# wgurecky/CORRLA_RS

Hardware: AMD Instinct MI355X
Metric: RSVD GFLOP/s on 16k x 16k f32 rank-128 (higher is better)
Workload: dtype f32

## Files before the change

### corrla_rs_amd/csrc/gemm_plan.hpp

```cpp
#pragma once
#include <algorithm>
#include <cstddef>
#include <cstdint>

#include "core_svd_plan.hpp"

namespace corrla {

constexpr int kMaxColTiles = 9;

struct ColBlocking {
  int tiles, nblk, nt;
  int64_t cols_alloc;
};
inline ColBlocking col_blocking(int64_t cols) {
  ColBlocking b;
  b.tiles = (int)std::max<int64_t>(1, (cols + 15) / 16);
  b.nblk = (b.tiles + kMaxColTiles - 1) / kMaxColTiles;
  b.nt = (b.tiles + b.nblk - 1) / b.nblk;
  b.cols_alloc = (int64_t)b.nblk * b.nt * 16;
  return b;
}

namespace k {

constexpr int kRowBytes = 256;
constexpr int kLoaders = 4;
CORRLA_HD constexpr int gemm_vec(int esz) { return 16 / esz; }
CORRLA_HD constexpr int gemm_kt(int esz) { return kRowBytes / esz; }
CORRLA_HD constexpr int outer_tile(int mw) { return 64 * mw; }
CORRLA_HD constexpr int big_tile_bytes(int mw) { return 64 * 256 * mw; }
CORRLA_HD constexpr int stage_bytes(int mw, int nt) { return big_tile_bytes(mw) + nt * 16 * kRowBytes; }
CORRLA_HD constexpr int gemm_stages(int mw, int nt) { return 3 * stage_bytes(mw, nt) <= 160 * 1024 ? 3 : 2; }
CORRLA_HD constexpr int gemm_lds_bytes(int mw, int nt) { return gemm_stages(mw, nt) * stage_bytes(mw, nt); }

template <class T>
CORRLA_HD constexpr int gram_rows() { return 512 / (int)sizeof(T); }
CORRLA_HD constexpr int gram_tile_bytes(int nct) { return 16 * nct * 512; }
CORRLA_HD constexpr int gram_stages(int nct) {
  const int s = (160 * 1024 - 4096) / gram_tile_bytes(nct);
  return s > 4 ? 4 : s;
}
CORRLA_HD constexpr int gram_lds_bytes(int nct, int esz) {
  const int ring = gram_stages(nct) * gram_tile_bytes(nct);
  const int red = 3 * (nct * (nct + 1) / 2) * 256 * esz;
  return ring > red ? ring : red;
}

constexpr int kMxWaves = 8;
constexpr int kMxLoaders = 4;
constexpr int kMxRowTiles = 2;
constexpr int kMxOuter = kMxWaves * kMxRowTiles * 16;
constexpr int kMxKT = 32;
constexpr int kMxBigBytes = kMxOuter * kMxKT * 4;
CORRLA_HD constexpr int mx_plane_bytes(int nt) { return nt * 16 * kMxKT * 2; }
constexpr int kMxASlots = 3, kMxBSlots = 2;
CORRLA_HD constexpr int mx_bslot_bytes(int nt, int np) { return np * mx_plane_bytes(nt); }
CORRLA_HD constexpr int mx_lds_bytes(int nt, int np) { return kMxASlots * kMxBigBytes + kMxBSlots * mx_bslot_bytes(nt, np) + 1024; }

}

struct GemmKnobs {
  int split_nn = 0, split_tn = 0;
  int mw = 0;
  int xcd_remap = 1;
  int64_t tall_min_rows = 65536;
  int persist_max_tiles = 16;
  int f64_waves = 8;
  double mixed_min_work = 16777216.0;
  bool even_blocks = false;
  bool no_gram_alias = false;
  bool no_rotate = false;
  int mixed_split = 0;
};

struct GemmOperand {
  int64_t rows = 0, cols = 0, ld = 0, cols_readable = 0, cols_alloc = 0;
  bool external = false, aligned = true;
};
struct GemmShape {
  bool tn = false;
  int esz = 4;
  GemmOperand r, x, out;
  bool same = false;
  int np = 0;
  int num_cus = 256;
};

enum class GemmFamily { general, gram_alias, tall_apply, tall_gram, bf16_split };
enum class SlabReduce { none, plain, deep };

struct SlabReducePlan {
  SlabReduce kind = SlabReduce::none;
  unsigned grid[2] = {0, 0};
  int slabs = 0;
  int64_t rows = 0, cols = 0;
};

struct GemmLaunch {
  unsigned grid[3] = {1, 1, 1};
  int nt = 0;
  int64_t col_base = 0;
  int xcd_remap = 0;
  int lds = 0;
};

struct GemmPlan {
  const char* error = nullptr;
  GemmFamily family = GemmFamily::general;
  int mw = 1, nw = 4, np = 0;
  int block = 256;
  int nlaunch = 0;
  GemmLaunch launch[2];
  int tiles_total = 0, nsplit = 1, tiles_per_split = 0, outer_blocks = 0, rotate = 0, vec_store = 0;
  int64_t out_cols = 0;
  int64_t slab_stride = 0;
  size_t slab_bytes = 0;
  SlabReducePlan reduce;
  int64_t rows_per_group = 0, groups = 0;
  int64_t plane_stride = 0, plane_cols = 0;
  size_t plane_bytes = 0;
  unsigned split_grid = 0;
};

inline bool gemm_mixed_domain(const GemmShape& s, const GemmKnobs& kn) {
  const int64_t outer_n = s.tn ? s.r.cols : s.r.rows, red_n = s.tn ? s.r.rows : s.r.cols;
  if (s.esz != 4 || s.x.external || col_blocking(s.x.cols).nblk != 1) return false;
  if (!s.r.aligned || (s.r.ld % 4) || (s.r.cols_readable % 4) || !s.x.aligned || (s.x.ld % 64)) return false;
  if (s.x.ld < (red_n + k::kMxKT - 1) / k::kMxKT * k::kMxKT || s.out.ld < outer_n || s.out.rows != outer_n) return false;
  if (s.same) return false;
  return outer_n >= 1 && red_n >= 1 && (double)outer_n * (double)red_n >= kn.mixed_min_work;
}

namespace gemm_plan_detail {

inline bool grid_fits(unsigned y, unsigned z) { return y <= 65535u && z <= 65535u; }
inline bool padding_fits(const GemmShape& s, const ColBlocking& cb) {
  return cb.cols_alloc <= s.x.cols_alloc && (s.out.external ? s.out.cols >= s.x.cols : cb.cols_alloc <= s.out.cols_alloc);
}
inline GemmPlan rejected(GemmPlan p, const char* why) {
  p.error = why;
  return p;
}

inline bool plan_reduce(GemmPlan& p, int64_t outer_n, int64_t cols_alloc) {
  if (p.nsplit <= 1) return true;
  const bool deep = p.nsplit >= 8;
  const unsigned rows_per_wg = deep ? 64 : 256;
  p.reduce = {deep ? SlabReduce::deep : SlabReduce::plain,
// ... 117 lines not shown
      nsplit = (int)((s.num_cus + wgs - 1) / wgs);
      if (wgs * nsplit < 2 * (int64_t)s.num_cus && wgs < s.num_cus / 4) nsplit *= 2;
      nsplit = std::min(nsplit, std::max(1, p.tiles_total / 4));
    }
    nsplit = std::min(std::max(1, std::min(nsplit, p.tiles_total)), 65535);
  }
  const int64_t outer_tiles = (outer_n + 64 * mw - 1) / (64 * mw);
  if (outer_tiles > 0x7fffffff) return rejected(p, "outer dimension too large");

  p.family = alias ? GemmFamily::gram_alias : GemmFamily::general;
  p.mw = mw == 2 ? 2 : 1;
  if (!alias && mw == 2 && s.esz == 8 && kn.f64_waves == 8) {
    p.mw = 1;
    p.nw = 8;
  }
  p.block = 64 * (p.nw + k::kLoaders);
  p.nsplit = nsplit;
  p.tiles_per_split = (p.tiles_total + nsplit - 1) / nsplit;
  p.outer_blocks = (int)outer_tiles;
  p.out_cols = s.out.external ? s.out.cols : (uneven ? (int64_t)cb.tiles * 16 : cb.cols_alloc);
  p.vec_store = ((s.out.ld % 4) == 0 && s.out.aligned) ? 1 : 0;
  p.rotate = (!s.tn && !alias && p.tiles_per_split <= 32 && p.tiles_per_split > 1 && !kn.no_rotate) ? 1 : 0;
  p.slab_stride = s.out.ld * cb.cols_alloc;
  if (nsplit > 1) p.slab_bytes = (size_t)nsplit * (size_t)p.slab_stride * s.esz;

  int64_t gx = outer_tiles;
  if (!alias && p.tiles_per_split <= kn.persist_max_tiles) {
    const int64_t lds_full = (int64_t)k::gemm_lds_bytes(mw, cb.nt);
    const int64_t per_cu = std::max<int64_t>(1, std::min<int64_t>(4, (160 * 1024) / lds_full));
    const int64_t slots = per_cu * s.num_cus / ((int64_t)cb.nblk * nsplit);
    if (slots >= 1 && outer_tiles >= 3 * slots) gx = slots;
  }
  if (!grid_fits((unsigned)cb.nblk, (unsigned)nsplit)) return rejected(p, "problem too large for the launch grid");

  const int gw = p.mw * p.nw / 4;
  p.nlaunch = uneven ? 2 : 1;
  for (int i = 0; i < p.nlaunch; ++i) {
    GemmLaunch& L = p.launch[i];
    L.grid[0] = (unsigned)gx;
    L.grid[1] = (unsigned)(uneven ? (i == 0 ? n_wide : cb.nblk - n_wide) : cb.nblk);
    L.grid[2] = (unsigned)nsplit;
    L.nt = cb.nt - i;
    L.col_base = (int64_t)i * n_wide * cb.nt * 16;
    L.xcd_remap = (s.tn && kn.xcd_remap && L.grid[1] == 1 && gx == outer_tiles && outer_tiles >= 2 && outer_tiles <= 32 &&
                   nsplit >= 8) ? 1 : 0;
    if (alias) {
      L.lds = 3 * k::big_tile_bytes(2);
    } else {
      const int64_t per_wg = (int64_t)std::max(1, p.tiles_per_split) * ((outer_tiles + gx - 1) / gx);
      L.lds = (int)std::min<int64_t>(k::gemm_stages(gw, L.nt), per_wg) * k::stage_bytes(gw, L.nt);
    }
  }
  if (!plan_reduce(p, outer_n, cb.cols_alloc)) p.error = "problem too large for the launch grid";
  return p;
}

}
```

### corrla_rs_amd/csrc/hip_backend.hpp

```cpp
#pragma once
#include <hip/hip_runtime.h>
#include <rccl/rccl.h>

#include <cmath>
#include <cstdio>
#include <cstdlib>
#include <cstring>
#include <limits>
#include <random>
#include <string>
#include <type_traits>
#include <vector>

#include "core_svd_plan.hpp"
#include "driver.hpp"
#include "hip_kernels.hpp"
#include "tsqr_kernels.hpp"
#include "jacobi_mc_kernels.hpp"
#include "ata_kernels.hpp"
#include "tall_kernels.hpp"
#include "mixed_kernels.hpp"
#include "grad_kernels.hpp"
#include "knn2_kernels.hpp"
#include "grad_wide_kernels.hpp"
// ... 29 lines not shown
struct NcclType<double> {
  static constexpr ncclDataType_t v = ncclDouble;
};

class HipDev {
 public:
  int device = 0;
  int num_cus = 256;
  hipStream_t stream = nullptr;
  ncclComm_t comm = nullptr;
  int comm_rank = 0, comm_size = 1;
  int n_collectives = 0;
  double collective_bytes = 0;

  explicit HipDev(int dev_ordinal) : device(dev_ordinal) {
    int count = 0;
    if (hipGetDeviceCount(&count) != hipSuccess || count <= 0)
      throw Error(ST_ENODEV, "no HIP device visible (libcorrla_rsvd has no CPU fallback)");
    if (dev_ordinal < 0 || dev_ordinal >= count) throw Error(ST_EINVAL, "device ordinal out of range");
    CORRLA_HIP(hipSetDevice(device));
    hipDeviceProp_t prop;
    CORRLA_HIP(hipGetDeviceProperties(&prop, device));
    if (std::strncmp(prop.gcnArchName, "gfx950", 6) != 0)
      throw Error(ST_ENODEV, std::string("device is ") + prop.gcnArchName + ", this library is built for gfx950 only");
    num_cus = prop.multiProcessorCount;
    CORRLA_HIP(hipStreamCreateWithFlags(&stream, hipStreamNonBlocking));
    CORRLA_HIP(hipMalloc(&zero_page_, 256));
    CORRLA_HIP(hipHostMalloc(&pinned_, kPinnedBytes, hipHostMallocDefault));
    for (auto& e : events_) CORRLA_HIP(hipEventCreate(&e));
    CORRLA_HIP(hipMemsetAsync(zero_page_, 0, 256, stream));
    set_lds_limits();
    {
      std::random_device rd;
      entropy_ = ((uint64_t)rd() << 32) ^ (uint64_t)rd();
    }
    no_device_chol_ = env_int("CORRLA_HOST_CHOL", 0) != 0;
    jmc_min_l_ = env_int("CORRLA_JMC_MIN_L", 96);
    jmc_max_b_ = std::min(32, std::max(2, env_int("CORRLA_JMC_MAX_B", 24)));
    robust_passes_ = std::max(2, env_int("CORRLA_ROBUST_PASSES", 2));
    robust_qr_ = env_int("CORRLA_DEVICE_ROBUST_QR", 1) != 0;
    gemm_debug_flags_ = env_int("CORRLA_GEMM_DEBUG", 0);
    gemm_knobs_.split_nn = env_int("CORRLA_SPLIT_NN", 0);
    gemm_knobs_.split_tn = env_int("CORRLA_SPLIT_TN", 0);
    gemm_knobs_.mw = env_int("CORRLA_MW", 0);
    gemm_knobs_.xcd_remap = env_int("CORRLA_GEMM_XCD", 1);
    gemm_knobs_.tall_min_rows = env_int("CORRLA_TALL_MIN_ROWS", 65536);
    gemm_knobs_.persist_max_tiles = env_int("CORRLA_GEMM_PERSIST_TILES", 16);
    gemm_knobs_.f64_waves = env_int("CORRLA_F64_WAVES", 8);
    if (const char* e = std::getenv("CORRLA_MIXED_MIN_WORK")) gemm_knobs_.mixed_min_work = std::atof(e);
    gemm_knobs_.even_blocks = env_int("CORRLA_EVEN_BLOCKS", 0) != 0;
    gemm_knobs_.no_gram_alias = env_int("CORRLA_NO_GRAM_ALIAS", 0) != 0;
    gemm_knobs_.no_rotate = env_int("CORRLA_GEMM_NO_ROTATE", 0) != 0;
    gemm_knobs_.mixed_split = env_int("CORRLA_MIXED_SPLIT", 0);
  }
  ~HipDev() {
    (void)hipSetDevice(device);
    if (stream) (void)hipStreamSynchronize(stream);
    if (comm) (void)ncclCommDestroy(comm);
    for (auto& c : chunks_) (void)hipFree(c.p);
    for (auto& c : zchunks_) (void)hipFree(c.p);
    if (zero_page_) (void)hipFree(zero_page_);
    if (pinned_) (void)hipHostFree(pinned_);
    for (auto& e : events_)
      if (e) (void)hipEventDestroy(e);
    for (auto& e : ev_pool_) (void)hipEventDestroy(e);
    if (stream) (void)hipStreamDestroy(stream);
  }
  HipDev(const HipDev&) = delete;
  HipDev& operator=(const HipDev&) = delete;

  int nranks() const { return comm_size; }

  uint64_t fresh_seed(bool rank_invariant) {
    uint64_t z = (rank_invariant ? 0x5eedull : entropy_) + 0x9e3779b97f4a7c15ull * (uint64_t)(++(rank_invariant ? calls_sharded_ : calls_));
    z = (z ^ (z >> 30)) * 0xbf58476d1ce4e5b9ull;
    z = (z ^ (z >> 27)) * 0x94d049bb133111ebull;
    z ^= z >> 31;
    return z ? z : 0x5eedull;
  }

  void comm_init(const void* id128, int rank, int nranks_) {
    CORRLA_HIP(hipSetDevice(device));
    ncclUniqueId id;
    static_assert(sizeof(ncclUniqueId) <= CORRLA_UNIQUE_ID_BYTES, "unique id size");
    std::memcpy(&id, id128, sizeof(id));
    if (comm) {
      (void)ncclCommDestroy(comm);
      comm = nullptr;
    }
    CORRLA_NCCL(ncclCommInitRank(&comm, nranks_, id, rank));
    comm_rank = rank;
    comm_size = nranks_;
  }
  void comm_info(int* rank_out, int* nranks_out) {
    if (!comm) {
      *rank_out = 0;
      *nranks_out = 0;
      return;
    }
    CORRLA_NCCL(ncclCommUserRank(comm, rank_out));
    CORRLA_NCCL(ncclCommCount(comm, nranks_out));
  }

  void begin_call() {
    CORRLA_HIP(hipSetDevice(device));
    events_set_[0] = events_set_[1] = events_set_[2] = false;
    n_collectives = 0;
    collective_bytes = 0;
    marks_.clear();
    ev_used_ = 0;
    phase_mark(nullptr);
    for (auto& c : chunks_) c.used = 0;
    sp_scratch_ = nullptr;
    sp_scratch_bytes_ = 0;
    for (auto& c : zchunks_) {
      c.zeroed = std::min<size_t>(c.used, (size_t)256 << 20);
      c.used = 0;
      if (c.zeroed) CORRLA_HIP(hipMemsetAsync(c.p, 0, c.zeroed, stream));
    }
  }
  void end_call() { sync(); }
  void sync() { CORRLA_HIP(hipStreamSynchronize(stream)); }

  void* alloc_bytes(size_t bytes) {
    bytes = (bytes + 255) / 256 * 256;
    if (bytes == 0) bytes = 256;
    for (auto& c : chunks_)
      if (c.size - c.used >= bytes) {
        void* p = (char*)c.p + c.used;
        c.used += bytes;
        return p;
      }
    Chunk c;
    c.size = std::max<size_t>(bytes, (size_t)64 << 20);
    if (hipMalloc(&c.p, c.size) != hipSuccess) {
      (void)hipGetLastError();
      throw Error(ST_ENOMEM, "device allocation of " + std::to_string(c.size) + " bytes failed");
    }
    c.used = bytes;
    chunks_.push_back(c);
    return c.p;
  }
  void memset_zero(void* p, size_t bytes) { CORRLA_HIP(hipMemsetAsync(p, 0, bytes, stream)); }
  void* alloc_zeroed(size_t bytes) {
    bytes = (bytes + 255) / 256 * 256;
    if (bytes == 0) bytes = 256;
    Chunk* hit = nullptr;
    for (auto& c : zchunks_)
      if (c.size - c.used >= bytes) {
        hit = &c;
        break;
      }
    if (!hit) {
      Chunk c;
      c.size = std::max<size_t>(bytes, (size_t)128 << 20);
      if (hipMalloc(&c.p, c.size) != hipSuccess) {
        (void)hipGetLastError();
        throw Error(ST_ENOMEM, "device allocation of " + std::to_string(c.size) + " bytes failed");
      }
      zchunks_.push_back(c);
      hit = &zchunks_.back();
    }
    char* p = (char*)hit->p + hit->used;
    const size_t end = hit->used + bytes;
    if (end > hit->zeroed) {
      const size_t from = std::max(hit->used, hit->zeroed);
      CORRLA_HIP(hipMemsetAsync((char*)hit->p + from, 0, end - from, stream));
    }
    hit->used = end;
    return p;
  }

  template <class T>
  Skinny<T> alloc_skinny(int64_t rows, int64_t cols) {
    Skinny<T> s;
    s.rows = rows;
    s.cols = cols;
    s.ld = round_up(std::max<int64_t>(rows, 1), kLdPad);
    s.cols_alloc = col_blocking(cols).cols_alloc;
    const size_t bytes = (size_t)s.ld * (size_t)s.cols_alloc * sizeof(T);
    s.p = (T*)alloc_zeroed(bytes);
    return s;
  }
  template <class T>
  Skinny<T> alloc_skinny_out(int64_t rows, int64_t cols) {
    Skinny<T> s;
    s.rows = rows;
    s.cols = cols;
    s.ld = round_up(std::max<int64_t>(rows, 1), kLdPad);
    s.cols_alloc = col_blocking(cols).cols_alloc;
    const size_t bytes = (size_t)s.ld * (size_t)s.cols_alloc * sizeof(T);
    if (bytes < ((size_t)4 << 20)) {
      s.p = (T*)alloc_zeroed(bytes);
      return s;
// ... 941 lines not shown
        continue;
      }
      if (marks_[i].slot) *marks_[i].slot += (double)ms;
    }
    if (total && marks_.size() >= 2) {
      float ms = 0.f;
      if (hipEventElapsedTime(&ms, marks_.front().ev, marks_.back().ev) == hipSuccess)
        *total = (double)ms;
      else
        (void)hipGetLastError();
    }
    marks_.clear();
  }

  void event_mark(int i) {
    CORRLA_HIP(hipEventRecord(events_[i], stream));
    events_set_[i] = true;
  }
  double event_elapsed_ms(int i, int j) {
    if (!events_set_[i] || !events_set_[j]) return 0.0;
    float ms = 0.f;
    if (hipEventElapsedTime(&ms, events_[i], events_[j]) != hipSuccess) {
      (void)hipGetLastError();
      return 0.0;
    }
    return (double)ms;
  }

  template <class F>
  double time_on_stream(int reps, F&& f) {
    hipEvent_t e0, e1;
    CORRLA_HIP(hipEventCreate(&e0));
    CORRLA_HIP(hipEventCreate(&e1));
    f();
    CORRLA_HIP(hipEventRecord(e0, stream));
    for (int i = 0; i < reps; ++i) f();
    CORRLA_HIP(hipEventRecord(e1, stream));
    CORRLA_HIP(hipEventSynchronize(e1));
    float ms = 0.f;
    CORRLA_HIP(hipEventElapsedTime(&ms, e0, e1));
    (void)hipEventDestroy(e0);
    (void)hipEventDestroy(e1);
    return (double)ms / reps;
  }

 private:
  struct Chunk {
    void* p = nullptr;
    size_t size = 0, used = 0;
    size_t zeroed = 0;
  };
  std::vector<Chunk> chunks_;
  std::vector<Chunk> zchunks_;
  void* sp_scratch_ = nullptr;
  size_t sp_scratch_bytes_ = 0;
  void* zero_page_ = nullptr;
  void* pinned_ = nullptr;
  hipEvent_t events_[3] = {nullptr, nullptr, nullptr};
  bool events_set_[3] = {false, false, false};
  struct PhaseMark {
    hipEvent_t ev;
    double* slot;
  };
  std::vector<hipEvent_t> ev_pool_;
  size_t ev_used_ = 0;
  std::vector<PhaseMark> marks_;
  static constexpr size_t kPinnedBytes = (size_t)8 << 20;
  int gemm_debug_flags_ = 0;
  GemmKnobs gemm_knobs_;
  uint64_t entropy_ = 0, calls_ = 0, calls_sharded_ = 0;
  bool no_device_chol_ = false;
  int jmc_min_l_ = 96, jmc_max_b_ = 24, jmc_local_ = 1;
  const int* run_if_ = nullptr;
  bool phase_events_ = true;
  bool robust_qr_ = true;
  int robust_passes_ = 2;
  int jmc_extra_sweeps_ = 0, jmc_sweeps_hint_ = 0;
  bool jmc_force_v_ = false;

  static void check_grid(const dim3& g) {
    if (g.y > 65535u || g.z > 65535u) throw Error(ST_EINVAL, "problem too large for the launch grid");
  }

  static void lds_limit(const void* fn, size_t bytes) {
    CORRLA_HIP(hipFuncSetAttribute(fn, hipFuncAttributeMaxDynamicSharedMemorySize, (int)bytes));
  }
  static void set_lds_limits() {
    constexpr size_t kMax = k::kLdsMaxBytes;
    set_lds_limits_typed<float>();
    set_lds_limits_typed<double>();
    set_ata_limits<2>();
    set_ata_limits<4>();
    set_ata_limits<8>();
    set_mixed_limits<2, false>();
    set_mixed_limits<2, true>();
    set_mixed_limits<3, false>();
    set_mixed_limits<3, true>();
    lds_limit((const void*)k::knn_kernel, kMax);
    lds_limit((const void*)k::knn_mfma_kernel<4, 4>, kMax);
    lds_limit((const void*)k::knn_mfma_kernel<4, 8>, kMax);
    lds_limit((const void*)k::knn_mfma_kernel<4, 16>, kMax);
    lds_limit((const void*)k::knn_mfma_kernel<2, 4>, kMax);
    lds_limit((const void*)k::knn_mfma_kernel<2, 8>, kMax);
    lds_limit((const void*)k::knn_mfma_kernel<2, 16>, kMax);
    lds_limit((const void*)k::knn2_kernel<1>, k::k2_lds_bytes(1));
    lds_limit((const void*)k::knn2_kernel<2>, k::k2_lds_bytes(2));
// ... 86 lines not shown
  }
  template <class T>
  void slab_reduce(const SlabReducePlan& rp, const T* slab, int64_t stride, T* out, int64_t ld, const T* scale, const int* run_if) {
    if (rp.kind == SlabReduce::none) return;
    const dim3 grid(rp.grid[0], rp.grid[1]);
    if (rp.kind == SlabReduce::deep)
      hipLaunchKernelGGL((k::slab_reduce_deep_kernel<T>), grid, dim3(256), 0, stream, slab, stride, rp.slabs, out, ld, rp.rows,
                         rp.cols, scale, run_if);
    else
      hipLaunchKernelGGL((k::slab_reduce_kernel<T>), grid, dim3(256), 0, stream, slab, stride, rp.slabs, out, ld, rp.rows, rp.cols,
                         scale, run_if);
    CORRLA_HIP(hipGetLastError());
  }

  template <class T, int NT>
  void launch_general(bool tn, const GemmPlan& p, dim3 grid, dim3 block, int lds, const k::GemmArgs<T>& a) {
    with_nt<2>(p.mw, [&](auto mw) {
      with_nt<8, 4>(p.nw, [&](auto nw) {
        constexpr int MW = decltype(mw)::value, NW = decltype(nw)::value;
        if constexpr (NW == 4 || (NW == 8 && MW == 1 && std::is_same<T, double>::value)) {
          if (tn)
            hipLaunchKernelGGL((k::gemm_tn_kernel<T, MW, NT, NW>), grid, block, lds, stream, a);
          else
            hipLaunchKernelGGL((k::gemm_nn_kernel<T, MW, NT, false, NW>), grid, block, lds, stream, a);
        }
      });
    });
  }

  template <class T>
  void launch_gemm(bool tn, const Big<T>& r, const Skinny<T>& x, Skinny<T>& out, const T* scale_dev) {
    const GemmPlan p = plan_gemm(tn, r, x, out, 0);
    const GemmLaunch& L0 = p.launch[0];
    T* slab = p.reduce.kind != SlabReduce::none ? (T*)alloc_bytes(p.slab_bytes) : nullptr;
    if (p.family == GemmFamily::tall_apply) {
      const k::TallApplyArgs<T> g{r.p, r.cols, r.ld, (int)r.rows, x.p, x.ld, (int)x.cols, out.p, out.ld, (int)p.out_cols,
                                  scale_dev, p.vec_store, run_if_};
      with_nt<sizeof(T) == 4 ? 6 : 4>(L0.nt, [&](auto kt) {
        constexpr int K = decltype(kt)::value;
        hipLaunchKernelGGL((k::tall_apply_kernel<T, K, K>), dim3(L0.grid[0]), dim3(p.block), L0.lds, stream, g);
      });
    } else if (p.family == GemmFamily::tall_gram) {
      const k::TallGramArgs<T> g{x.p, r.cols, x.ld, (int)out.rows, slab, p.slab_stride, out.ld, p.rows_per_group,
                                 (const T*)zero_page_, run_if_};
      with_nt<sizeof(T) == 4 ? 6 : 4>(L0.nt, [&](auto nct) {
        hipLaunchKernelGGL((k::tall_gram_kernel<T, decltype(nct)::value>), dim3(L0.grid[0]), dim3(p.block), L0.lds, stream, g);
      });
    } else {
      k::GemmArgs<T> a{r.p, r.rows, r.cols, r.ld, r.cols_readable,
                       x.p, x.ld,
                       out.p, out.ld, p.out_cols, 0,
                       slab, p.slab_stride, scale_dev, (const T*)zero_page_,
                       p.tiles_total, p.tiles_per_split, p.nsplit, gemm_debug_flags_, run_if_,
                       p.vec_store, p.rotate, p.outer_blocks, 0};
      for (int i = 0; i < p.nlaunch; ++i) {
        const GemmLaunch& L = p.launch[i];
        const dim3 grid(L.grid[0], L.grid[1], L.grid[2]), block(p.block);
        a.col_base = L.col_base;
        a.xcd_remap = L.xcd_remap;
        if (p.family == GemmFamily::gram_alias)
          with_nt<8>(L.nt, [&](auto nt) {
            hipLaunchKernelGGL((k::gemm_nn_kernel<T, 2, decltype(nt)::value, true>), grid, block, L.lds, stream, a);
          });
        else
          with_nt<kMaxColTiles>(L.nt, [&](auto nt) { launch_general<T, decltype(nt)::value>(tn, p, grid, block, L.lds, a); });
      }
    }
    CORRLA_HIP(hipGetLastError());
    slab_reduce<T>(p.reduce, slab, p.slab_stride, out.p, out.ld, scale_dev, run_if_);
  }

  template <class T>
  void launch_copy_out(const T* src, int64_t lds_, int64_t rows, int64_t cols, T* dst, int64_t ldd, bool transpose) {
    const int64_t tiles_c = (cols + 31) / 32, tiles_r = (rows + 31) / 32;
    if (tiles_c * tiles_r > 0x7fffffff) throw Error(ST_EINVAL, "problem too large for the launch grid");
    dim3 grid((unsigned)(tiles_c * tiles_r));
    hipLaunchKernelGGL((k::copy_out_kernel<T>), grid, dim3(256), 0, stream, src, lds_, rows, cols, dst, ldd,
                       transpose ? 1 : 0, tiles_c);
    CORRLA_HIP(hipGetLastError());
  }
};

}
```

### corrla_rs_amd/csrc/hip_kernels.hpp

```cpp
#pragma once
#include <hip/hip_runtime.h>

#include <limits>
#include <stdint.h>

#include <type_traits>

#include "gemm_plan.hpp"

namespace corrla {
namespace k {

typedef float f32x4 __attribute__((ext_vector_type(4)));
typedef double f64x4 __attribute__((ext_vector_type(4)));
typedef double f64x2 __attribute__((ext_vector_type(2)));

#ifndef CORRLA_F32_BIG_IS_A
#define CORRLA_F32_BIG_IS_A true
#endif
template <class T>
struct MT;
template <>
struct MT<float> {
  typedef f32x4 acc_t;
// ... 8 lines not shown
  static __device__ __forceinline__ int tswz(int row) { return ((row >> 2) & 1) << 2; }
};
template <>
struct MT<double> {
  typedef f64x4 acc_t;
  typedef f64x2 vec_t;
  static constexpr int VEC = gemm_vec(8);
  static constexpr int KT = gemm_kt(8);
  static constexpr bool kBigIsA = false;
  static __device__ __forceinline__ acc_t mma(double a, double b, acc_t c) {
    return __builtin_amdgcn_mfma_f64_16x16x4f64(a, b, c, 0, 0, 0);
  }
  static __device__ __forceinline__ int drow(int lane, int j) { return (lane >> 4) + 4 * j; }
  static __device__ __forceinline__ int tswz(int row) { return ((row >> 1) & 1) << 3; }
};

#ifndef CORRLA_PD
#define CORRLA_PD 4
#endif
#ifndef CORRLA_GEMM_DEFER
#define CORRLA_GEMM_DEFER 2
#endif
constexpr int kPrefetchSteps = CORRLA_PD;
template <int N>
__device__ __forceinline__ void wait_vmcnt() {
  static_assert(N >= 0 && N <= 63, "vmcnt is a 6-bit counter");
  asm volatile("s_waitcnt vmcnt(%0)" ::"n"(N) : "memory");
}
__device__ __forceinline__ void wg_barrier() { asm volatile("s_barrier" ::: "memory"); }

template <class T>
struct GemmArgs {
  const T* r;
  int64_t r_rows, r_cols, r_ld, r_cols_readable;
  const T* x;
  int64_t x_ld;
  T* out;
  int64_t out_ld;
  int64_t out_cols;
  int64_t col_base;
  T* slab;
  int64_t slab_stride;
  const T* scale;
  const T* zero;
  int tiles_total;
  int tiles_per_split;
  int nsplit;
  int debug_flags;
  const int* run_if;
  int vec_store;
  int rotate;
  int outer_blocks;
  int xcd_remap;
};

__device__ __forceinline__ void glds16(const void* gsrc, char* lds_wave_base) {
  __builtin_amdgcn_global_load_lds((const __attribute__((address_space(1))) void*)gsrc,
                                   (__attribute__((address_space(3))) void*)lds_wave_base, 16, 0, 0);
}


template <int I, int N, class F>
__device__ __forceinline__ void static_for(F&& f) {
  if constexpr (I < N) {
    f(std::integral_constant<int, I>{});
    static_for<I + 1, N>(f);
  }
}

template <int NVAR, int NQ, int CS>
struct DmaStream {
  const char* ptr[NVAR];
  int64_t step;
  int64_t adv;
  __device__ __forceinline__ void issue(char* lds) {
    static_for<0, NQ>([&](auto iq) {
      static_for<0, NVAR>([&](auto ip) {
        constexpr int q = decltype(iq)::value, pv = decltype(ip)::value;
        glds16(ptr[pv], lds + CS * (pv + NVAR * q) * 1024);
        ptr[pv] += step;
      });
    });
    const int64_t back = adv - (int64_t)NQ * step;
#pragma unroll
    for (int pv = 0; pv < NVAR; ++pv) ptr[pv] += back;
  }
};

template <int OFF, class V>
__device__ __forceinline__ void lds_read_b128(V& d, unsigned addr) {
  static_assert(sizeof(V) == 16 && OFF >= 0 && OFF < 65536, "ds_read_b128 operand");
  asm volatile("ds_read_b128 %0, %1 offset:%2" : "=v"(d) : "v"(addr), "n"(OFF) : "memory");
}
template <int OFF>
__device__ __forceinline__ void lds_read_elem(float& d, unsigned addr) {
  static_assert(OFF >= 0 && OFF < 65536, "ds_read_b32 offset");
  asm volatile("ds_read_b32 %0, %1 offset:%2" : "=v"(d) : "v"(addr), "n"(OFF) : "memory");
}
template <int OFF>
__device__ __forceinline__ void lds_read_elem(double& d, unsigned addr) {
  static_assert(OFF >= 0 && OFF < 65536, "ds_read_b64 offset");
  asm volatile("ds_read_b64 %0, %1 offset:%2" : "=v"(d) : "v"(addr), "n"(OFF) : "memory");
}
template <int N, class V>
__device__ __forceinline__ void lds_wait(V& frag) {
  static_assert(N >= 0 && N <= 15, "lgkmcnt is a 4-bit counter");
// ... 13 lines not shown
    return MT<T>::mma(r, x, c);
  else
    return MT<T>::mma(x, r, c);
}

template <class T, int NT>
__device__ __forceinline__ void store_tile(const GemmArgs<T>& g, const typename MT<T>::acc_t (&acc)[NT], int64_t outer0,
                                           int64_t outer_limit, int64_t col0, int lane, int slab_z = (int)blockIdx.z) {
  if (g.debug_flags & 8) return;
  T* dst;
  T sc = (T)1;
  if (g.nsplit > 1) {
    dst = g.slab + (int64_t)slab_z * g.slab_stride;
  } else {
    dst = g.out;
    if (g.scale) {
      sc = *g.scale;
      asm volatile("" : "+v"(sc));
    }
  }
  if constexpr (MT<T>::kBigIsA) {
    const int64_t outer = outer0 + 4 * (lane >> 4);
    if (outer >= outer_limit) return;
    const bool whole = g.vec_store && outer + 3 < outer_limit;
#pragma unroll
    for (int t = 0; t < NT; ++t) {
      const int64_t col = col0 + 16 * t + (lane & 15);
      if (g.nsplit > 1 || col < g.out_cols) {
        T* p = dst + col * g.out_ld + outer;
        if (whole) {
          *(typename MT<T>::acc_t*)p = acc[t] * sc;
        } else {
#pragma unroll
          for (int j = 0; j < 4; ++j)
            if (outer + j < outer_limit) p[j] = acc[t][j] * sc;
        }
      }
    }
  } else {
    const int64_t outer = outer0 + (lane & 15);
    if (outer >= outer_limit) return;
    static_assert(sizeof(T) == 8, "the scalar-store epilogue is the f64 layout (drow = (lane >> 4) + 4 j)");
    const int64_t colb = col0 + (lane >> 4);
    T* p = dst + colb * g.out_ld + outer;
    const int64_t step = 4 * g.out_ld;
#pragma unroll
    for (int t = 0; t < NT; ++t) {
#pragma unroll
      for (int j = 0; j < 4; ++j) {
        const int64_t col = colb + 16 * t + 4 * j;
        if (g.nsplit > 1 || col < g.out_cols) *p = acc[t][j] * sc;
        p += step;
      }
    }
  }
}

template <class T, int MW, int NT, bool ALIAS = false, int NW = 4>
__global__ __launch_bounds__(64 * (NW + kLoaders)) void gemm_nn_kernel(GemmArgs<T> g) {
  constexpr int GW = MW * NW / 4;
  static_assert(NW == 4 || (NW == 8 && !ALIAS), "4 or 8 MFMA waves");
  typedef typename MT<T>::acc_t acc_t;
  typedef typename MT<T>::vec_t vec_t;
  constexpr int VEC = MT<T>::VEC;
  constexpr int KT = MT<T>::KT;
  constexpr int STAGE = ALIAS ? big_tile_bytes(GW) : stage_bytes(GW, NT);
  constexpr int BIG = big_tile_bytes(GW);
  static_assert(!ALIAS || 16 * NT <= 64 * GW, "alias: the outer tile must hold every column");
  extern __shared__ __attribute__((aligned(16))) char smem[];
  if (g.run_if && *g.run_if == 0) return;
  const int lane = threadIdx.x & 63;
  const int wave = __builtin_amdgcn_readfirstlane(threadIdx.x >> 6);
  const int64_t row_first = (int64_t)blockIdx.x * outer_tile(GW);
  const int64_t col0 = g.col_base + (int64_t)blockIdx.y * (NT * 16);
  const int t_begin = blockIdx.z * g.tiles_per_split;
  const int t_end = min(t_begin + g.tiles_per_split, g.tiles_total);
  const int nk = t_end - t_begin;
  const int nob = (g.outer_blocks - (int)blockIdx.x + (int)gridDim.x - 1) / (int)gridDim.x;
  const int64_t ob_rows = (int64_t)gridDim.x * outer_tile(GW);

  if (wave >= NW) {
    __builtin_amdgcn_s_setprio(3);
    int64_t row0 = row_first;
    auto stage_checked = [&](int buf, int kt) {
      char* rt = smem + buf * STAGE;
      const int64_t k0 = (int64_t)kt * KT;
      for (int c = wave - NW; c < (ALIAS ? 4 * NT : 16 * GW); c += kLoaders) {
        const int row = 4 * c + (lane >> 4);
        const int ls = (lane & 15) ^ (row & 15);
        const int64_t grow = row0 + row;
        const int64_t kk = k0 + ls * VEC;
        const T* src = (grow < g.r_rows && kk < g.r_cols_readable) ? g.r + grow * g.r_ld + kk : g.zero;
        glds16(src, rt + c * 1024);
      }
      if constexpr (!ALIAS)
        for (int c = wave - NW; c < 4 * NT; c += kLoaders) {
          const int row = 4 * c + (lane >> 4);
          const int ls = (lane & 15) ^ (row & 15);
          glds16(g.x + (col0 + row) * g.x_ld + k0 + ls * VEC, rt + BIG + c * 1024);
        }
    };
    constexpr int NL = kLoaders, NV = 4 / NL;
    const int lw = wave - NW;
    DmaStream<NV, ALIAS ? NT : 4 * GW, NL> big;
    DmaStream<NV, NT, NL> sk;
    const int rot = g.rotate ? (int)(blockIdx.x % (unsigned)nk) : 0;
// ... 115 lines not shown
          lds_read_b128<mw * 16 * kRowBytes>(bfr[gq][mw], b_off[gq] + sb);
        });
      }
      lds_read_b128<t * 16 * kRowBytes>(afr[st], a_off[gq] + sb);
    };
    static_for<0, (PD < NS ? PD : NS)>(read_step);
    if constexpr (kDefer > 0) {
      if (have_prev) {
        static_for<0, kDefer>([&](auto id) {
          constexpr int d = decltype(id)::value;
          constexpr int t = (NS - kDefer + d) % NT;
          lds_tie(da[d]);
#pragma unroll
          for (int mw = 0; mw < MW; ++mw)
#pragma unroll
            for (int j = 0; j < VEC; ++j) acc[mw][t] = gemm_mma<T>(da[d][j], db[mw][j], acc[mw][t]);
        });
      }
    }
    static_for<0, NS>([&](auto ic) {
      constexpr int st = decltype(ic)::value;
      constexpr int gq = st / NT, t = st % NT;
      if constexpr (st + PD < NS) read_step(std::integral_constant<int, st + PD>{});
      constexpr int last = (st + PD < NS) ? st + PD : NS - 1;
      constexpr int groups = last / NT - gq;
      constexpr int younger = (last - st) + groups * MW;
      lds_wait<(younger < 15 ? younger : 15)>(afr[st]);
      if constexpr (t == 0) {
        static_for<0, MW>([&](auto im) { lds_tie(bfr[gq][decltype(im)::value]); });
      }
      if constexpr (st < NS - kDefer) mfma_step(ic);
    });
  };

  constexpr int NSTAGE_C = ALIAS ? 3 : gemm_stages(GW, NT);
  int buf = 0;
  int64_t row0 = row_first;
  for (int ob = 0; ob < nob; ++ob, row0 += ob_rows) {
#pragma unroll
    for (int mw = 0; mw < MW; ++mw)
#pragma unroll
      for (int t = 0; t < NT; ++t) acc[mw][t] = (acc_t){0, 0, 0, 0};
    for (int i = 0; i < nk; ++i) {
      wg_barrier();
      compute(buf, i > 0);
      buf = buf + 1 == NSTAGE_C ? 0 : buf + 1;
    }
    if constexpr (kDefer > 0) {
      if (nk > 0) static_for<NS - kDefer, NS>(mfma_step);
    }
#pragma unroll
    for (int mw = 0; mw < MW; ++mw)
      store_tile<T, NT>(g, acc[mw], row0 + 16 * MW * wave + 16 * mw, g.r_rows, col0, lane);
  }
}

template <class T, int MW, int NT, int NW = 4>
__global__ __launch_bounds__(64 * (NW + kLoaders)) void gemm_tn_kernel(GemmArgs<T> g) {
  constexpr int GW = MW * NW / 4;
  static_assert(NW == 4 || NW == 8, "4 or 8 MFMA waves");
  typedef typename MT<T>::acc_t acc_t;
  typedef typename MT<T>::vec_t vec_t;
  constexpr int VEC = MT<T>::VEC;
  constexpr int KT = MT<T>::KT;
  constexpr int STAGE = stage_bytes(GW, NT);
  constexpr int BIG = big_tile_bytes(GW);
  constexpr int RBT = 64 * GW * (int)sizeof(T);
  constexpr int LPR = RBT / 16;
  extern __shared__ __attribute__((aligned(16))) char smem[];
  if (g.run_if && *g.run_if == 0) return;
  const int lane = threadIdx.x & 63;
  const int wave = __builtin_amdgcn_readfirstlane(threadIdx.x >> 6);
  int bx = (int)blockIdx.x, bz = (int)blockIdx.z;
  if (g.xcd_remap) {
    const int gx = (int)gridDim.x, per = 8 * gx;
    const int lin = bx + gx * bz, grp = lin / per, r = lin - grp * per;
    if ((grp + 1) * 8 <= (int)gridDim.z) {
      bx = r >> 3;
      bz = grp * 8 + (r & 7);
    }
  }
  const int64_t n_first = (int64_t)bx * outer_tile(GW);
  const int64_t col0 = g.col_base + (int64_t)blockIdx.y * (NT * 16);
  const int t_begin = bz * g.tiles_per_split;
  const int t_end = min(t_begin + g.tiles_per_split, g.tiles_total);
  const int nk = t_end - t_begin;
  const int nob = (g.outer_blocks - bx + (int)gridDim.x - 1) / (int)gridDim.x;
  const int64_t ob_cols = (int64_t)gridDim.x * outer_tile(GW);

  if (wave >= NW) {
    __builtin_amdgcn_s_setprio(3);
    int64_t n0 = n_first;
    auto stage_checked = [&](int buf, int mt) {
      char* rt = smem + buf * STAGE;
      const int64_t m0 = (int64_t)mt * KT;
      for (int c = wave - NW; c < 16 * GW; c += kLoaders) {
        const int lin = c * 64 + lane;
        const int row = lin / LPR;
        const int lsb = (lin % LPR) ^ MT<T>::tswz(row);
        const int64_t grow = m0 + row;
        const int64_t nn = n0 + (int64_t)lsb * VEC;
        const T* src = (grow < g.r_rows && nn < g.r_cols_readable) ? g.r + grow * g.r_ld + nn : g.zero;
        glds16(src, rt + c * 1024);
      }
      for (int c = wave - NW; c < 4 * NT; c += kLoaders) {
        const int row = 4 * c + (lane >> 4);
// ... 113 lines not shown
          constexpr int mw = decltype(iq)::value / VEC, j = decltype(iq)::value % VEC;
          lds_read_elem<(4 * gq * VEC + j) * RBT>(bfr[gq][mw][j], b_off[mw] + sb);
        });
      }
      lds_read_b128<t * 16 * kRowBytes>(afr[st], a_off[gq] + sb);
    };
    static_for<0, (PD < NS ? PD : NS)>(read_step);
    if constexpr (kDefer > 0) {
      if (have_prev) {
        static_for<0, kDefer>([&](auto id) {
          constexpr int d = decltype(id)::value;
          constexpr int t = (NS - kDefer + d) % NT;
          lds_tie(da[d]);
#pragma unroll
          for (int mw = 0; mw < MW; ++mw)
#pragma unroll
            for (int j = 0; j < VEC; ++j) acc[mw][t] = gemm_mma<T>(da[d][j], db[mw][j], acc[mw][t]);
        });
      }
    }
    static_for<0, NS>([&](auto ic) {
      constexpr int st = decltype(ic)::value;
      constexpr int gq = st / NT, t = st % NT;
      if constexpr (st + PD < NS) read_step(std::integral_constant<int, st + PD>{});
      constexpr int last = (st + PD < NS) ? st + PD : NS - 1;
      constexpr int groups = last / NT - gq;
      constexpr int younger = (last - st) + groups * MW * VEC;
      lds_wait<(younger < 15 ? younger : 15)>(afr[st]);
      if constexpr (t == 0) {
        static_for<0, MW * VEC>([&](auto iq) { lds_tie(bfr[gq][decltype(iq)::value / VEC][decltype(iq)::value % VEC]); });
      }
      if constexpr (st < NS - kDefer) mfma_step(ic);
    });
  };

  int buf = 0;
  int64_t n0 = n_first;
  for (int ob = 0; ob < nob; ++ob, n0 += ob_cols) {
#pragma unroll
    for (int mw = 0; mw < MW; ++mw)
#pragma unroll
      for (int t = 0; t < NT; ++t) acc[mw][t] = (acc_t){0, 0, 0, 0};
    for (int i = 0; i < nk; ++i) {
      wg_barrier();
      compute(buf, i > 0);
      buf = buf + 1 == gemm_stages(GW, NT) ? 0 : buf + 1;
    }
    if constexpr (kDefer > 0) {
      if (nk > 0) static_for<NS - kDefer, NS>(mfma_step);
    }
#pragma unroll
    for (int mw = 0; mw < MW; ++mw)
      store_tile<T, NT>(g, acc[mw], n0 + 16 * MW * wave + 16 * mw, g.r_cols, col0, lane, bz);
  }
}

template <class T>
__global__ void slab_reduce_kernel(const T* slab, int64_t slab_stride, int nsplit, T* out, int64_t ld, int64_t limit,
                                   int64_t ncols, const T* scale, const int* run_if = nullptr) {
  if (run_if && *run_if == 0) return;
  const int64_t i = (int64_t)blockIdx.x * blockDim.x + threadIdx.x;
  const int64_t col = blockIdx.y;
  if (i >= limit || col >= ncols) return;
  const int64_t off = col * ld + i;
  T s = 0;
  for (int z = 0; z < nsplit; ++z) s += slab[(int64_t)z * slab_stride + off];
  if (scale) s *= *scale;
  out[off] = s;
}
template <class T>
__global__ __launch_bounds__(256) void slab_reduce_deep_kernel(const T* slab, int64_t slab_stride, int nsplit, T* out,
                                                               int64_t ld, int64_t limit, int64_t ncols, const T* scale,
                                                               const int* run_if = nullptr) {
  if (run_if && *run_if == 0) return;
  __shared__ T part[4][64];
  const int li = threadIdx.x & 63, zg = threadIdx.x >> 6;
  const int64_t i = (int64_t)blockIdx.x * 64 + li;
  const int64_t col = blockIdx.y;
  const int per = (nsplit + 3) / 4;
  const int z0 = zg * per, z1 = min(nsplit, z0 + per);
  T s0 = 0, s1 = 0, s2 = 0, s3 = 0;
  if (i < limit && col < ncols) {
    const T* src = slab + col * ld + i;
    int z = z0;
    for (; z + 3 < z1; z += 4) {
      s0 += src[(int64_t)z * slab_stride];
      s1 += src[(int64_t)(z + 1) * slab_stride];
      s2 += src[(int64_t)(z + 2) * slab_stride];
      s3 += src[(int64_t)(z + 3) * slab_stride];
    }
    for (; z < z1; ++z) s0 += src[(int64_t)z * slab_stride];
  }
  part[zg][li] = (s0 + s1) + (s2 + s3);
  __syncthreads();
  if (zg == 0 && i < limit && col < ncols) {
    T s = (part[0][li] + part[1][li]) + (part[2][li] + part[3][li]);
    if (scale) s *= *scale;
    out[col * ld + i] = s;
  }
}

template <class T>
__global__ void sumsq_partial_kernel(const T* y, int64_t n, double* partial) {
  double s = 0.0;
  for (int64_t i = (int64_t)blockIdx.x * blockDim.x + threadIdx.x; i < n; i += (int64_t)gridDim.x * blockDim.x) {
    const double v = (double)y[i];
// ... 1261 lines not shown
```

Before: 92000.

## Fuse split-K slab reduction into GEMM kernels via per-wave arrival tickets

Split-K GEMM waves now take an atomic ticket after storing their partial slab. The last-arriving wave for each output tile sums all slabs and writes the final, scaled output, so the separate slab_reduce kernel launch is skipped when the plan enables it (plain reductions by default). This removes a kernel launch and a second pass over the slab. In exchange it adds release/acquire fences and atomics per wave, leaves a serialized reduction tail on the last wave, and needs a persistent zeroed ticket buffer that must reset to zero after every use.

Result: slower. 87050 (-5.4%).

```diff
diff --git a/corrla_rs_amd/csrc/gemm_plan.hpp b/corrla_rs_amd/csrc/gemm_plan.hpp
--- a/corrla_rs_amd/csrc/gemm_plan.hpp
+++ b/corrla_rs_amd/csrc/gemm_plan.hpp
@@ -72,6 +72,7 @@
   bool no_gram_alias = false;
   bool no_rotate = false;
   int mixed_split = 0;
+  int slab_inkernel = 1;
 };
 
 struct GemmOperand {
@@ -95,6 +96,8 @@
   unsigned grid[2] = {0, 0};
   int slabs = 0;
   int64_t rows = 0, cols = 0;
+  bool in_kernel = false;
+  int64_t tickets = 0;
 };
 
 struct GemmLaunch {
@@ -318,6 +321,11 @@
     }
   }
   if (!plan_reduce(p, outer_n, cb.cols_alloc)) p.error = "problem too large for the launch grid";
+  if (p.reduce.kind != SlabReduce::none &&
+      (kn.slab_inkernel >= 2 || (kn.slab_inkernel == 1 && p.reduce.kind == SlabReduce::plain))) {
+    p.reduce.in_kernel = true;
+    p.reduce.tickets = (int64_t)p.outer_blocks * cb.nblk * p.nw;
+  }
   return p;
 }
 
diff --git a/corrla_rs_amd/csrc/hip_backend.hpp b/corrla_rs_amd/csrc/hip_backend.hpp
--- a/corrla_rs_amd/csrc/hip_backend.hpp
+++ b/corrla_rs_amd/csrc/hip_backend.hpp
@@ -105,6 +105,7 @@
     gemm_knobs_.no_gram_alias = env_int("CORRLA_NO_GRAM_ALIAS", 0) != 0;
     gemm_knobs_.no_rotate = env_int("CORRLA_GEMM_NO_ROTATE", 0) != 0;
     gemm_knobs_.mixed_split = env_int("CORRLA_MIXED_SPLIT", 0);
+    gemm_knobs_.slab_inkernel = env_int("CORRLA_SLAB_INKERNEL", 1);
   }
   ~HipDev() {
     (void)hipSetDevice(device);
@@ -112,6 +113,7 @@
     if (comm) (void)ncclCommDestroy(comm);
     for (auto& c : chunks_) (void)hipFree(c.p);
     for (auto& c : zchunks_) (void)hipFree(c.p);
+    for (auto& c : tickets_) (void)hipFree(c.p);
     if (zero_page_) (void)hipFree(zero_page_);
     if (pinned_) (void)hipHostFree(pinned_);
     for (auto& e : events_)
@@ -172,7 +174,16 @@
       if (c.zeroed) CORRLA_HIP(hipMemsetAsync(c.p, 0, c.zeroed, stream));
     }
   }
-  void end_call() { sync(); }
+  void end_call() {
+    sync();
+    if (!tickets_.empty() && env_int("CORRLA_DEBUG", 0)) {
+      const Chunk& c = tickets_.back();
+      std::vector<unsigned> h(c.size / sizeof(unsigned));
+      CORRLA_HIP(hipMemcpy(h.data(), c.p, c.size, hipMemcpyDeviceToHost));
+      for (size_t i = 0; i < h.size(); ++i)
+        if (h[i]) throw Error(ST_EHIP, "internal: split-sum ticket " + std::to_string(i) + " left at " + std::to_string(h[i]));
+    }
+  }
   void sync() { CORRLA_HIP(hipStreamSynchronize(stream)); }
 
   void* alloc_bytes(size_t bytes) {
@@ -193,6 +204,20 @@
     c.used = bytes;
     chunks_.push_back(c);
     return c.p;
+  }
+  unsigned* split_tickets(int64_t n) {
+    const size_t bytes = (size_t)std::max<int64_t>(n, 1) * sizeof(unsigned);
+    if (tickets_.empty() || tickets_.back().size < bytes) {
+      Chunk c;
+      c.size = std::max<size_t>((bytes + 4095) / 4096 * 4096, (size_t)64 << 10);
+      if (hipMalloc(&c.p, c.size) != hipSuccess) {
+        (void)hipGetLastError();
+        throw Error(ST_ENOMEM, "device allocation of " + std::to_string(c.size) + " bytes failed");
+      }
+      CORRLA_HIP(hipMemsetAsync(c.p, 0, c.size, stream));
+      tickets_.push_back(c);
+    }
+    return (unsigned*)tickets_.back().p;
   }
   void memset_zero(void* p, size_t bytes) { CORRLA_HIP(hipMemsetAsync(p, 0, bytes, stream)); }
   void* alloc_zeroed(size_t bytes) {
@@ -1240,6 +1265,7 @@
   };
   std::vector<Chunk> chunks_;
   std::vector<Chunk> zchunks_;
+  std::vector<Chunk> tickets_;
   void* sp_scratch_ = nullptr;
   size_t sp_scratch_bytes_ = 0;
   void* zero_page_ = nullptr;
@@ -1432,7 +1458,8 @@
                        out.p, out.ld, p.out_cols, 0,
                        slab, p.slab_stride, scale_dev, (const T*)zero_page_,
                        p.tiles_total, p.tiles_per_split, p.nsplit, gemm_debug_flags_, run_if_,
-                       p.vec_store, p.rotate, p.outer_blocks, 0};
+                       p.vec_store, p.rotate, p.outer_blocks, 0,
+                       p.reduce.in_kernel ? split_tickets(p.reduce.tickets) : nullptr};
       for (int i = 0; i < p.nlaunch; ++i) {
         const GemmLaunch& L = p.launch[i];
         const dim3 grid(L.grid[0], L.grid[1], L.grid[2]), block(p.block);
@@ -1447,7 +1474,7 @@
       }
     }
     CORRLA_HIP(hipGetLastError());
-    slab_reduce<T>(p.reduce, slab, p.slab_stride, out.p, out.ld, scale_dev, run_if_);
+    if (!p.reduce.in_kernel) slab_reduce<T>(p.reduce, slab, p.slab_stride, out.p, out.ld, scale_dev, run_if_);
   }
 
   template <class T>
diff --git a/corrla_rs_amd/csrc/hip_kernels.hpp b/corrla_rs_amd/csrc/hip_kernels.hpp
--- a/corrla_rs_amd/csrc/hip_kernels.hpp
+++ b/corrla_rs_amd/csrc/hip_kernels.hpp
@@ -84,6 +84,7 @@
   int rotate;
   int outer_blocks;
   int xcd_remap;
+  unsigned* tickets;
 };
 
 __device__ __forceinline__ void glds16(const void* gsrc, char* lds_wave_base) {
@@ -203,6 +204,84 @@
         if (g.nsplit > 1 || col < g.out_cols) *p = acc[t][j] * sc;
         p += step;
       }
+    }
+  }
+}
+
+__device__ __forceinline__ bool split_arrive_last(unsigned* ticket, int nsplit, int lane) {
+  asm volatile("s_waitcnt vmcnt(0)" ::: "memory");
+  __builtin_amdgcn_fence(__ATOMIC_RELEASE, "agent");
+  asm volatile("s_waitcnt vmcnt(0)" ::: "memory");
+  unsigned t = 0;
+  if (lane == 0) t = atomicAdd(ticket, 1u);
+  t = __builtin_amdgcn_readfirstlane(t);
+  if (t != (unsigned)nsplit - 1u) return false;
+  if (lane == 0) __hip_atomic_store(ticket, 0u, __ATOMIC_RELAXED, __HIP_MEMORY_SCOPE_AGENT);
+  __builtin_amdgcn_fence(__ATOMIC_ACQUIRE, "agent");
+  asm volatile("s_waitcnt vmcnt(0)" ::: "memory");
+  return true;
+}
+template <class V, class T>
+__device__ __forceinline__ V slab_sum(const T* src, int64_t stride, int nsplit) {
+  auto at = [&](int z) { return *(const V*)(src + (int64_t)z * stride); };
+  if (nsplit < 8) {
+    V s{};
+#pragma unroll 1
+    for (int z = 0; z < nsplit; ++z) s += at(z);
+    return s;
+  }
+  const int per = (nsplit + 3) / 4;
+  auto group = [&](int zg) {
+    const int z0 = zg * per, z1 = min(nsplit, z0 + per);
+    V s0{}, s1{}, s2{}, s3{};
+    int z = z0;
+#pragma unroll 1
+    for (; z + 3 < z1; z += 4) {
+      s0 += at(z);
+      s1 += at(z + 1);
+      s2 += at(z + 2);
+      s3 += at(z + 3);
+    }
+#pragma unroll 1
+    for (; z < z1; ++z) s0 += at(z);
+    return (s0 + s1) + (s2 + s3);
+  };
+  const V p0 = group(0), p1 = group(1), p2 = group(2), p3 = group(3);
+  return (p0 + p1) + (p2 + p3);
+}
+template <class T>
+__device__ __noinline__ void split_finish(unsigned* ticket, const T* slab, int64_t slab_stride, int nsplit, T* out, int64_t out_ld,
+                                          int64_t out_cols, const T* scale, int vec_store, int64_t outer0, int rows,
+                                          int64_t outer_limit, int64_t col0, int ncols) {
+  typedef typename MT<T>::vec_t vec_t;
+  constexpr int VEC = MT<T>::VEC;
+  static_assert(sizeof(vec_t) == 16, "16-byte vectors");
+  const int lane = threadIdx.x & 63;
+  if (!split_arrive_last(ticket, nsplit, lane)) return;
+  if (outer0 >= outer_limit) return;
+  T sc = (T)1;
+  if (scale) sc = *scale;
+  if (vec_store && outer0 + rows <= outer_limit) {
+    const int rv = rows / VEC;
+    const int r = (lane % rv) * VEC;
+#pragma unroll 1
+    for (int c = lane / rv; c < ncols; c += 64 / rv) {
+      const int64_t col = col0 + c;
+      if (col >= out_cols) break;
+      const int64_t off = col * out_ld + outer0 + r;
+      vec_t s = slab_sum<vec_t, T>(slab + off, slab_stride, nsplit);
+      if (scale) s *= sc;
+      *(vec_t*)(out + off) = s;
+    }
+  } else {
+#pragma unroll 1
+    for (int e = lane; e < rows * ncols; e += 64) {
+      const int64_t row = outer0 + e % rows, col = col0 + e / rows;
+      if (row >= outer_limit || col >= out_cols) continue;
+      const int64_t off = col * out_ld + row;
+      T s = slab_sum<T, T>(slab + off, slab_stride, nsplit);
+      if (scale) s *= sc;
+      out[off] = s;
     }
   }
 }
@@ -424,6 +503,11 @@
 #pragma unroll
     for (int mw = 0; mw < MW; ++mw)
       store_tile<T, NT>(g, acc[mw], row0 + 16 * MW * wave + 16 * mw, g.r_rows, col0, lane);
+    if (g.tickets) {
+      const int64_t tk = ((int64_t)(blockIdx.x + ob * gridDim.x) * gridDim.y + blockIdx.y) * NW + wave;
+      split_finish<T>(g.tickets + tk, g.slab, g.slab_stride, g.nsplit, g.out, g.out_ld, g.out_cols, g.scale, g.vec_store,
+                      row0 + 16 * MW * wave, 16 * MW, g.r_rows, col0, 16 * NT);
+    }
   }
 }
 
@@ -643,6 +727,11 @@
 #pragma unroll
     for (int mw = 0; mw < MW; ++mw)
       store_tile<T, NT>(g, acc[mw], n0 + 16 * MW * wave + 16 * mw, g.r_cols, col0, lane, bz);
+    if (g.tickets) {
+      const int64_t tk = ((int64_t)(bx + ob * (int)gridDim.x) * gridDim.y + blockIdx.y) * NW + wave;
+      split_finish<T>(g.tickets + tk, g.slab, g.slab_stride, g.nsplit, g.out, g.out_ld, g.out_cols, g.scale, g.vec_store,
+                      n0 + 16 * MW * wave, 16 * MW, g.r_cols, col0, 16 * NT);
+    }
   }
 }
 
```
